# Harounnn/Clustering-Driven-Replication-Strategy

Hardware: AMD Instinct MI355X
Metric: Lloyd point-iters/sec (whole node) + achieved HBM GB/s, 100M files d=16 k=64 (higher is better)
Workload: dtype f64

## Files before the change

clustering-driven-replication-strategy_amd/_cdr.py:

```python
from __future__ import annotations

import ctypes
import os
import sys
import threading

import numpy as np

_HERE = os.path.dirname(os.path.abspath(__file__))
LIB_PATH = os.environ.get("CDR_LIB", os.path.join(_HERE, "libcdr.so"))

CDR_OK = 0
CDR_ERR_ARG = 1
CDR_ERR_HIP = 2
CDR_ERR_NAN = 3
CDR_ERR_STATE = 4
CDR_ERR_UNSUPPORTED = 5
MODE_F32X = 1
MODE_F64 = 2
SEED_BLOCK = 8192
PLAN_SLOT = 64
PLAN_MAX_TAIL = PLAN_SLOT - 1
PLAN_MAX_FIELD = 65535

# ... 7 lines not shown
_PF64 = ctypes.POINTER(ctypes.c_double)

SIGNATURES = {
    "cdr_last_error": ([], ctypes.c_char_p),
    "cdr_version": ([], ctypes.c_int),
    "cdr_device_count": ([ctypes.POINTER(ctypes.c_int)], None),
    "cdr_create": ([ctypes.c_int, ctypes.POINTER(_P)], None),
    "cdr_destroy": ([_P], None),
    "cdr_set_stream": ([_P, _P], None),
    "cdr_synchronize": ([_P], None),
    "cdr_points_load_f64": ([_P, _P, _I64, _I32], None),
    "cdr_points_generate": ([_P, _I64, _I64, _I64, _I32, _I32, _U64], None),
    "cdr_points_info": ([_P, _PI64, _PI32, _PI32, _PI32], None),
    "cdr_points_get_rows": ([_P, _P, _I64, _P], None),
    "cdr_points_stats": ([_P, _P], None),
    "cdr_points_restat": ([_P, _P, _I64], None),
    "cdr_seed_reset": ([_P], None),
    "cdr_seed_update": ([_P, _P], None),
    "cdr_seed_num_blocks": ([_P, _PI64], None),
    "cdr_seed_block_sums": ([_P, _P], None),
    "cdr_seed_scan": ([_P, _F64, _F64, _PF64], None),
    "cdr_seed_search": ([_P, _F64, _F64, _PI64], None),
    "cdr_seed_scan_begin": ([_P, _F64, _F64, _PI64, _PI64], None),
    "cdr_seed_scan_items": ([_P, _P, _I64, _PI64], None),
    "cdr_seed_scan_end": ([_P, _F64, _PF64], None),
    "cdr_seed_program_eval": ([_P, _I64, _F64, _PF64, _PI32], None),
    "cdr_seed_stats": ([_P, _PI64], None),
    "cdr_seed_run": ([_P, _I64, _I32, _P, _P], None),
    "cdr_seed_shard_begin": ([_P, _I64, _I64, _I32, _I32, _I64, _I32, _P, _P, _P], None),
    "cdr_seed_shard_phase": ([_P, _I32, _P, _P], None),
    "cdr_seed_shard_end": ([_P, _P, _P, _P, _P], None),
    "cdr_seed_run_sharded": ([_P, _I64, _I64, _I64, _I32, _P, _P, _P, _P], None),
    "cdr_lloyd_step": ([_P, _P, _I32, _P, _I32], None),
    "cdr_lloyd_step_f64": ([_P, _P, _I32, _P, _P], None),
    "cdr_lloyd_f64_run": ([_P, _P, _I32, _I32, _F64, _P, _P, _P, _P], None),
    "cdr_lloyd_step_f32r": ([_P, _P, _I32, _P, _P], None),
    "cdr_f32r_seed_update": ([_P, _P, _I32, _P], None),
    "cdr_f32r_seed_run": ([_P, _I64, _I32, _P, _P], None),
    "cdr_lloyd_labels": ([_P, _P], None),
    "cdr_lloyd_stats": ([_P, _PI64], None),
    "cdr_debug_screen": ([_P, _P, _I32, _P, _P], None),
    "cdr_debug_plan32": ([_P, _I32, _P, _I32, _P], None),
    "cdr_profile_reset": ([_P, _I32], None),
    "cdr_profile_read": ([_P, _P], None),
    "cdr_profile_read_sub": ([_P, _P], None),
    "cdr_f64s_begin": ([_P, _P, _I32, _I32, _I32, _P, _P], None),
    "cdr_f64s_build": ([_P, _P, _P], None),
    "cdr_f64s_finish": ([_P, _P, _P, _P, _P, _P], None),
    "cdr_f64s_chain": ([_P, _P], None),
    "cdr_profile_kernel": ([_P, _P, _I32], None),
    "cdr_lloyd_screen_layout": ([_P, _P], None),
    "cdr_lloyd_watch_info": ([_P, _P], None),
    "cdr_debug_watch": ([_P, _P, _I64, _P, _I64, _P, _P], None),
    "cdr_lloyd_big_layout": ([_P, _P], None),
    "cdr_debug_big_plan": ([_P, _I32, _P, _I64, _PI64], None),
    "cdr_points_sqdev": ([_P, _P, _PF64], None),
    "cdr_lloyd_begin": ([_P, _P, _I32, _F64, _I32, _P, _F64], None),
    "cdr_lloyd_enqueue_assign": ([_P, _P], None),
    "cdr_lloyd_enqueue_finalize": ([_P, _P], None),
    "cdr_lloyd_status": ([_P, _P, _P], None),
    "cdr_lloyd_read": ([_P, _P, _P, _P], None),
    "cdr_lloyd_resume": ([_P, _P, _I32, _I32], None),
    "cdr_lloyd_end": ([_P], None),
    "cdr_lloyd_enqueue_steps": ([_P, _I32], None),
    "cdr_comm_unique_id": ([_P], None),
    "cdr_comm_init": ([_P, _P, _I32, _I32], None),
    "cdr_comm_destroy": ([_P], None),
    "cdr_comm_available": ([ctypes.POINTER(ctypes.c_int32)], None),
    "cdr_comm_ranks": ([_P, ctypes.POINTER(ctypes.c_int32), ctypes.POINTER(ctypes.c_int32)], None),
    "cdr_build_id": ([], ctypes.c_char_p),
    "cdr_medians_segmented": ([_P, _P, _P, _I64, _P], None),
    "cdr_medians_by_label": ([_P, _I32, _P], None),
    "cdr_features_aggregate": ([_P, _I64, _P, _P, _P, _P, _I64, _P, _P, _PI64], None),
    "cdr_features_finalize": ([_P, _I64, _P, _P, _F64, _P], None),
    "cdr_features_generate": ([_P, _I64, _I64, ctypes.c_uint64, _I64, _I64], None),
    "cdr_features_aggregate_resident": ([_P, _P, _PI64], None),
    "cdr_features_events_read": ([_P, _P, _P, _P, _P, _P], None),
    "cdr_features_groupby_info": ([_P, _P], None),
    "cdr_lloyd_f64_walked": ([_P, _PI64], None),
    "cdr_medians_group": ([_P, _I32, _P], None),
    "cdr_medians_begin": ([_P, _P, ctypes.POINTER(ctypes.c_int32), _PI64], None),
    "cdr_medians_pass_hist": ([_P, _I32, _P], None),
    "cdr_medians_pass_select": ([_P, _I32, _P], None),
    "cdr_medians_finish": ([_P, _P], None),
    "cdr_medians_global": ([_P, _P], None),
    "cdr_medians_global_begin": ([_P, _I64, ctypes.POINTER(ctypes.c_int32), _PI64], None),
    "cdr_medians_global_pass_hist": ([_P, _I32, _P], None),
    "cdr_medians_global_pass_select": ([_P, _I32, _P], None),
    "cdr_medians_global_finish": ([_P, _P], None),
    "cdr_medians_global_timing": ([_P, _P], None),
    "cdr_features_exchange_pack": ([_P, _I32, _P, _P, _P, _PI64], None),
    "cdr_features_exchange_unpack": ([_P, _P, _I64, _I64, _I64], None),
    "cdr_features_load_events": ([_P, _I64, _P, _P, _P, _P, _I64, _P], None),
    "cdr_features_finalize_stats": ([_P, _I64, _P, _P, ctypes.c_double, _P, _P], None),
    "cdr_features_finalize_apply": ([_P, _I64, _P, _P, ctypes.c_double, _P, _P, _I64, _P],
                                    None),
    "cdr_features_simulate": ([_P, _I64, _I64, ctypes.c_double, _I32, ctypes.c_uint64, _I64,
                               _PI64], None),
    "cdr_ingest_manifest": ([_P, _I64, _P, _P, _P, _I32, _P, _P], None),
    "cdr_ingest_log": ([_P, _P, _I64, _P], None),
    "cdr_ingest_reparse": ([_P, _P], None),
    "cdr_quality_silhouette": ([_P, _P, _I64, _P, _I32, _P, _P, _P], None),
    "cdr_quality_scatter": ([_P, _P, _I32, _P, _P, _P], None),
    "cdr_quality_timing": ([_P, _P], None),
    "cdr_csv_format": ([_P, _I64, _I32, ctypes.c_uint32, _P, _P, _P, _P, _I64, _PI64, _P, _I64,
                        _PI64], None),
# ... 384 lines not shown
        out = np.empty(self.info()["n"], dtype=np.int64)
        _check(self._lib.cdr_lloyd_labels(self._h, _ptr(out)))
        return out

    def fallback_count(self) -> int:
        v = _I64()
        _check(self._lib.cdr_lloyd_stats(self._h, ctypes.byref(v)))
        return int(v.value)

    def profile_reset(self, enable: bool = True, every: int = 1) -> None:
        _check(self._lib.cdr_profile_reset(self._h, max(int(every), 1) if enable else 0))

    def profile_read(self) -> dict:
        out = np.zeros(6, dtype=np.float64)
        _check(self._lib.cdr_profile_read(self._h, _ptr(out)))
        return {"screen_ms": out[0], "steps": int(out[1]), "step_ms": out[2],
                "fallback_points": int(out[3]), "queued_points": int(out[4]),
                "tight_points": int(out[5])}

    def profile_read_sub(self) -> dict:
        out = np.zeros(2, dtype=np.float64)
        _check(self._lib.cdr_profile_read_sub(self._h, _ptr(out)))
        return {"first_ms": out[0], "steps": int(out[1])}

    def profile_kernel(self) -> str:
        buf = ctypes.create_string_buffer(96)
        _check(self._lib.cdr_profile_kernel(self._h, buf, 96))
        return buf.value.decode()

    def screen_layout(self) -> dict:
        out = np.zeros(6, dtype=np.int32)
        _check(self._lib.cdr_lloyd_screen_layout(self._h, _ptr(out)))
        names = ("workgroups", "slot_wg", "dyn_pct", "max_chunks", "nchunks", "word_bytes")
        return {nm: int(v) for nm, v in zip(names, out)}

    def watch_info(self) -> dict:
        out = np.zeros(12, dtype=np.int64)
        _check(self._lib.cdr_lloyd_watch_info(self._h, _ptr(out)))
        names = ("mode", "listed", "failed", "epochs", "full_steps", "list_steps", "waves",
                 "range", "cap", "next_list", "carried", "n_pad")
        return {nm: int(v) for nm, v in zip(names, out)}

    def debug_watch(self) -> dict:
        info = self.watch_info()
        words = np.zeros(info["n_pad"], dtype=np.uint16)
        entries = np.zeros((info["waves"], info["cap"]), dtype=np.uint32)
        counts = np.zeros(info["waves"], dtype=np.int32)
        tables = np.zeros((3, 64), dtype=np.uint32)
        _check(self._lib.cdr_debug_watch(self._h, _ptr(words), words.size, _ptr(entries),
                                         entries.size, _ptr(counts), _ptr(tables)))
        return {"words": words, "entries": entries, "counts": counts, "T": tables[0],
                "H": tables[1], "HL": tables[2], **info}

    def big_layout(self) -> dict:
        out = np.zeros(15, dtype=np.int64)
        _check(self._lib.cdr_lloyd_big_layout(self._h, _ptr(out)))
        names = ("DQ", "KB", "FG", "JB", "l1_threads", "l2_form", "delta", "plan", "regions",
                 "cap1", "groups", "leftovers", "l3", "mv1", "mv2")
        return {nm: int(v) for nm, v in zip(names, out)}

    def debug_big_plan(self, k: int) -> dict:
        d = self.info()["d"]
        dq, kb = -(-d // 16), -(-int(k) // 32)
        b1, bc, bC = kb * dq * 64 * 16, kb * 32 * 4, 8 * int(k) * d
        got = _I64()
        _check(self._lib.cdr_debug_big_plan(self._h, int(k), None, 0, ctypes.byref(got)))
        if got.value != b1 + bc + bC + 16:
            raise RuntimeError(f"debug_big_plan: {got.value} bytes, expected {b1 + bc + bC + 16}")
        raw = np.empty(got.value, dtype=np.uint8)
        _check(self._lib.cdr_debug_big_plan(self._h, int(k), _ptr(raw), raw.size,
                                            ctypes.byref(got)))
        return {"frag1": raw[:b1].copy(), "cinit": raw[b1:b1 + bc].copy(),
                "C": raw[b1 + bc:b1 + bc + bC].copy().view(np.float64).reshape(int(k), d),
                "thr": raw[b1 + bc + bC:b1 + bc + bC + 8].copy().view(np.float32)}

    LL_RUNNING, LL_CONVERGED, LL_EMPTY, LL_HOST_PLAN, LL_AMBIGUOUS = 0, 1, 2, 3, 4

    def points_sqdev(self, ref) -> float:
        ref = np.ascontiguousarray(ref, dtype=np.float64)
        v = _F64()
        _check(self._lib.cdr_points_sqdev(self._h, _ptr(ref), ctypes.byref(v)))
        return float(v.value)

    def lloyd_begin(self, C, tol: float, ref, x2_total: float = float("nan"),
                    round32: bool = False) -> None:
        C = np.ascontiguousarray(C, dtype=np.float64)
        ref = np.ascontiguousarray(ref, dtype=np.float64)
        self._ll_shape = C.shape
        _check(self._lib.cdr_lloyd_begin(self._h, _ptr(C), C.shape[0], float(tol),
                                         1 if round32 else 0, _ptr(ref), float(x2_total)))

    def lloyd_enqueue_assign(self, dsums_ptr: int | None = None) -> None:
        _check(self._lib.cdr_lloyd_enqueue_assign(self._h, _P(dsums_ptr or 0)))

    def lloyd_enqueue_finalize(self, dsums_ptr: int | None = None) -> None:
        _check(self._lib.cdr_lloyd_enqueue_finalize(self._h, _P(dsums_ptr or 0)))

    def lloyd_status(self) -> dict:
        st = np.zeros(4, dtype=np.int64)
        v = np.zeros(2, dtype=np.float64)
        _check(self._lib.cdr_lloyd_status(self._h, _ptr(st), _ptr(v)))
        return {"running": bool(st[0]), "steps": int(st[1]), "reason": int(st[2]),
                "enqueued": int(st[3]), "shift": float(v[0]), "inertia": float(v[1])}

    def lloyd_read(self):
        k, d = self._ll_shape
# ... 588 lines not shown
```

clustering-driven-replication-strategy_amd/csrc/loop.hip:

```cpp
#include <cmath>
#include <cstdio>
#include <cstring>

#include "cdr_internal.h"
#include "fin32.h"
#include "plan32.h"

namespace cdr {

constexpr int kLLState = 8;

void plan32_point_side(const Ctx& c, double& xxmax, double& l1x);
void zh_rebase(Ctx& c, const long long* gate);
constexpr int kRebaseEvery = 4;

constexpr int kFinThreads = 512;
constexpr int kFinLds = 64 * 17;

__global__ __launch_bounds__(kFinThreads) void ll_finalize(FinArgs a) {
  long long* __restrict__ state = a.state;
  const int k = a.k, d = a.d;
  double* __restrict__ C = a.C;
  double* __restrict__ Cnew = a.Cnew;
  const int cells = k * (d + 1);
  __shared__ long long lsum[kFinLds];
  __shared__ double lC[kFinLds];
  __shared__ double lref[2 * 64];
  const bool staged = cells <= kFinLds && d <= 64;
  const double* __restrict__ ref = staged ? lref : a.ref;
  const double* __restrict__ Cin = staged ? lC : C;
  if (staged) {
    constexpr int PER = (kFinLds + kFinThreads - 1) / kFinThreads;
    long long p[PER][kRunSlices];
    double cv[PER];
    double rv = 0.0;
    const long long st0 = state[0];
#pragma unroll
    for (int i = 0; i < PER; ++i) {
      const int c = threadIdx.x + i * kFinThreads;
#pragma unroll
      for (int sl = 0; sl < kRunSlices; ++sl)
        p[i][sl] = (c < cells && sl < a.nslices) ? a.sums[(size_t)sl * cells + c] : 0;
      cv[i] = c < k * d ? C[c] : 0.0;
    }
    if (threadIdx.x < 2 * d) rv = a.ref[threadIdx.x];
    if (st0 == 0) return;
#pragma unroll
    for (int i = 0; i < PER; ++i) {
      const int c = threadIdx.x + i * kFinThreads;
      long long v = 0;
#pragma unroll
      for (int sl = 0; sl < kRunSlices; ++sl) v += p[i][sl];
      if (c < cells) lsum[c] = v;
      if (c < k * d) lC[c] = cv[i];
    }
    if (threadIdx.x < 2 * d) lref[threadIdx.x] = rv;
    __syncthreads();
  } else if (state[0] == 0) {
    return;
  }
  auto sum_at = [&](size_t e) -> long long {
    if (staged) return lsum[e];
    long long v = 0;
    for (int sl = 0; sl < a.nslices; ++sl) v += a.sums[(size_t)sl * cells + e];
    return v;
  };
// ... 483 lines not shown
  int wh[16];
  HIP_CHECK(hipMemcpy(wh, static_cast<unsigned char*>(c.bnd.p) + kBndWatch, sizeof(wh),
                      hipMemcpyDeviceToHost));
  std::vector<int32_t> wn((size_t)c.watch_waves), wf((size_t)c.watch_waves);
  HIP_CHECK(hipMemcpy(wn.data(), c.wn.p, sizeof(int32_t) * wn.size(), hipMemcpyDeviceToHost));
  HIP_CHECK(hipMemcpy(wf.data(), c.wf.p, sizeof(int32_t) * wf.size(), hipMemcpyDeviceToHost));
  const bool any = wh[kWListN] + wh[kWFullN] > 0;
  out[0] = any ? wh[kWLast] : -1;
  if (wh[kWEpochs] > 0)
    for (int32_t v : wn) out[1] += v;
  if (any)
    for (int32_t v : wf) out[2] += v;
  out[3] = wh[kWEpochs];
  out[4] = wh[kWFullN];
  out[5] = wh[kWListN];
  out[6] = c.watch_waves;
  out[7] = c.watch_range;
  out[8] = c.watch_cap;
  out[9] = wh[kWMode] == kWatchList && wh[kWOvf] == 0 ? 1 : 0;
  out[10] = wh[kWCarried];
  CDR_CATCH
}

int cdr_debug_watch(cdr_ctx* h, uint16_t* words, int64_t n_words, uint32_t* entries,
                    int64_t n_entries, int32_t* counts, uint32_t* tables) {
  CDR_TRY
  if (!h) CDR_FAIL(CDR_ERR_ARG, "null ctx");
  Ctx& c = h->c;
  if (!c.watch_on || !c.zb_valid || c.zb_fmt != 16)
    CDR_FAIL(CDR_ERR_STATE, "watch list: the list path is not on");
  if ((words && n_words != c.n_pad) ||
      (entries && n_entries != (int64_t)c.watch_waves * c.watch_cap))
    CDR_FAIL(CDR_ERR_ARG, "watch list: buffer sizes differ from cdr_lloyd_watch_info's");
  HIP_CHECK(hipSetDevice(c.device));
  HIP_CHECK(hipStreamSynchronize(c.stream));
  if (words)
    HIP_CHECK(hipMemcpy(words, c.zb.p, sizeof(uint16_t) * (size_t)c.n_pad, hipMemcpyDeviceToHost));
  if (entries)
    HIP_CHECK(hipMemcpy(entries, c.wl.p,
                        sizeof(uint32_t) * (size_t)c.watch_waves * (size_t)c.watch_cap,
                        hipMemcpyDeviceToHost));
  if (counts)
    HIP_CHECK(hipMemcpy(counts, c.wn.p, sizeof(int32_t) * (size_t)c.watch_waves,
                        hipMemcpyDeviceToHost));
  if (tables) {
    const unsigned char* bt = static_cast<const unsigned char*>(c.bnd.p);
    HIP_CHECK(hipMemcpy(tables, bt + kBndT, 256, hipMemcpyDeviceToHost));
    HIP_CHECK(hipMemcpy(tables + 64, bt + kBndH, 256, hipMemcpyDeviceToHost));
    HIP_CHECK(hipMemcpy(tables + 128, bt + kBndHL, 256, hipMemcpyDeviceToHost));
  }
  CDR_CATCH
}

int cdr_lloyd_end(cdr_ctx* h) {
  CDR_TRY
  if (!h) CDR_FAIL(CDR_ERR_ARG, "null ctx");
  h->c.ll_on = false;
  CDR_CATCH
}

}
```

clustering-driven-replication-strategy_amd/csrc/screen32_common.h:

```cpp
#pragma once
#include <type_traits>
#include <cstdio>
#include <cmath>
#include <cstring>
#include <algorithm>
#include <vector>

#include "cdr_internal.h"
#include "exact_math.h"
#include "plan32.h"

namespace cdr {

typedef _Float16 h8 __attribute__((ext_vector_type(8)));
typedef _Float16 h16 __attribute__((ext_vector_type(16)));
typedef float f4 __attribute__((ext_vector_type(4)));
typedef float f16v __attribute__((ext_vector_type(16)));
typedef _Float16 h2 __attribute__((ext_vector_type(2)));

__device__ __forceinline__ unsigned pack_h2(float a, float b) {
  h2 h = {(_Float16)a, (_Float16)b};
  return __builtin_bit_cast(unsigned, h);
}

// ... 213 lines not shown
  const float s = (l0 - u0) + w;
  const float m = 0x1p-21f * ((l0 + u0) + w);
  const float z = s - m;
  return (z > 0.0f ? (__float_as_uint(z) & ~63u) : 0xBF800000u) | label;
}

__device__ __forceinline__ unsigned short zb16_pack(float l0, float u0, float w, int e0,
                                                    unsigned label) {
  if (!(l0 > 0.0f) || !(u0 >= 0.0f) || !(w >= 0.0f)) return (unsigned short)label;
  l0 = fminf(l0, 0x1p60f) * (1.0f - 0x1p-20f);
  const float s = (l0 - u0) + w;
  const float m = 0x1p-21f * ((l0 + u0) + w);
  int c = zb16_code(s - m, e0);
  c = c < 0 ? 0 : (c > 1022 ? 1022 : c);
  return (unsigned short)((unsigned)c << 6 | label);
}


template <int QMAX, class F>
inline void dispatch_q_mt(int Q, int MT, F&& f) {
  static_assert(QMAX == 2 || QMAX == 4, "feature quads: 1..2 per lane half or 1..4 per point");
  if (Q < 1 || Q > QMAX || MT < 1 || MT > 2)
    CDR_FAIL(CDR_ERR_STATE, "screen32: no kernel for this (Q, MT)");
  auto with_q = [&](auto q) {
    if (MT == 1) f(q, std::integral_constant<int, 1>{});
    else f(q, std::integral_constant<int, 2>{});
  };
  if constexpr (QMAX == 4) {
    if (Q == 3) return with_q(std::integral_constant<int, 3>{});
    if (Q == 4) return with_q(std::integral_constant<int, 4>{});
  }
  if (Q == 1) with_q(std::integral_constant<int, 1>{});
  else with_q(std::integral_constant<int, 2>{});
}

template <class K>
inline int occupancy_blocks(K kernel, size_t lds) {
  int nb = 0;
  if (hipOccupancyMaxActiveBlocksPerMultiprocessor(&nb, kernel, 256, lds) != hipSuccess || nb < 1)
    nb = 2;
  return nb > 8 ? 8 : nb;
}

int screen32_blocks_per_cu(int QH, int MT, size_t lds);
void screen32_launch(int QH, int MT, dim3 grid, hipStream_t s, size_t lds, const S32Args& a);
int screen32p_blocks_per_cu(int Q, int MT);
void screen32p_launch(int Q, int MT, dim3 grid, hipStream_t s, const S32PArgs& p);
int screen32b_blocks_per_cu(int Q, int MT);
void screen32b_launch(int Q, int MT, dim3 grid, hipStream_t s, const S32BArgs& p);
void screen32bz_launch(dim3 grid, hipStream_t s, const S32BArgs& p);
void bound_words_reset(bool z16, hipStream_t s, const uint8_t* lab8, void* zb, int64_t n,
                       int64_t n_pad, const long long* gate);
void zh_rebase(Ctx& c, const long long* gate);
int screen32bs_blocks_per_cu(int Q, int MT, bool list);
void screen32bs_launch(int Q, int MT, dim3 grid, hipStream_t s, const S32BArgs& p, bool split);

}
```

clustering-driven-replication-strategy_amd/csrc/screen32b.hip:

```cpp
#include "screen32_common.h"
#include "screen32_fix.h"

namespace cdr {

template <int Q, int MT>
__global__ __launch_bounds__(256, 4) void screen32b(S32BArgs B) {
  const S32PArgs& a = B.p;
  constexpr int QH = FixDims<Q>::QH;
  if (a.gate && a.gate[0] == 0) return;
  constexpr bool H1 = QH == 1;
  constexpr int kTile = H1 ? 512 : 1024;
  constexpr int kHalf = kTile / 2;
  constexpr int kPB = H1 ? 8 : 16;
  constexpr int NWH = kPB / 4;
  constexpr int kRow = 2 * kPB;
  typedef unsigned u4v __attribute__((ext_vector_type(4)));
  __shared__ __attribute__((aligned(16))) float c32s[64 * kPrStr + 128];
  float* const eb = c32s + 64 * kPrStr;
  float* const hc = eb + 64;
  constexpr size_t kQBytes = 4 * 2 * 2 * kTile + 4 * 128 * sizeof(int2);
  __shared__ __attribute__((aligned(16))) unsigned char qlds[kQBytes > kFixLdsBytes ? kQBytes : kFixLdsBytes];
  typedef unsigned char QRow[2][2 * kTile];
  QRow* qd = reinterpret_cast<QRow*>(qlds);
  int2 (*qm)[128] = reinterpret_cast<int2 (*)[128]>(qlds + 4 * 2 * 2 * kTile);
// ... 383 lines not shown
  if (lane < cnt) out[total + lane] = fl[lane];
  if (lane == 0) B.zn[wave] = total + cnt;
}

__global__ void zb_reset_kernel(const uint8_t* __restrict__ lab8, uint32_t* __restrict__ zb,
                                int64_t n, int64_t n_pad, const long long* __restrict__ gate) {
  if (gate && gate[0] == 0) return;
  for (int64_t i = (int64_t)blockIdx.x * blockDim.x + threadIdx.x; i < n_pad;
       i += (int64_t)gridDim.x * blockDim.x)
    zb[i] = i < n ? (kZbStale | lab8[i]) : 0x7F000000u;
}

__global__ void zh_reset_kernel(const uint8_t* __restrict__ lab8, uint16_t* __restrict__ zh,
                                int64_t n, int64_t n_pad, const long long* __restrict__ gate) {
  if (gate && gate[0] == 0) return;
  for (int64_t i = (int64_t)blockIdx.x * blockDim.x + threadIdx.x; i < n_pad;
       i += (int64_t)gridDim.x * blockDim.x)
    zh[i] = i < n ? (uint16_t)lab8[i] : (uint16_t)kZ16Pad;
}

__device__ __forceinline__ unsigned zb16_rebase(unsigned w, float dg, int e0o, int e0n) {
  const unsigned c = w >> 6;
  if (c == 0u || c == 1023u) return w;
  const float t = zb16_dec((int)c, e0o) - dg;
  int cn = t > 0.0f ? zb16_code(t * (1.0f - 0x1p-22f), e0n) : -1;
  cn = cn < 0 ? 0 : (cn > 1022 ? 1022 : cn);
  return (unsigned)cn << 6 | (w & 63u);
}

__global__ __launch_bounds__(256) void zh_rebase_kernel(uint16_t* __restrict__ zh, int64_t n_pad,
                                                        const unsigned char* __restrict__ bt,
                                                        const long long* __restrict__ gate) {
  if (gate && gate[0] == 0) return;
  const int* hd = reinterpret_cast<const int*>(bt + kBndHdr);
  if (hd[3] == 0) return;
  __shared__ float dgs[64];
  if (threadIdx.x < 64) dgs[threadIdx.x] = reinterpret_cast<const float*>(bt + kBndDG)[threadIdx.x];
  __syncthreads();
  const int e0o = hd[1], e0n = hd[2];
  typedef unsigned u4v __attribute__((ext_vector_type(4)));
  u4v* z4 = reinterpret_cast<u4v*>(zh);
  for (int64_t i = (int64_t)blockIdx.x * blockDim.x + threadIdx.x; i < n_pad / 8;
       i += (int64_t)gridDim.x * blockDim.x) {
    u4v z = __builtin_nontemporal_load(z4 + i);
#pragma unroll
    for (int q = 0; q < 4; ++q) {
      const unsigned lo = z[q] & 0xFFFFu, hi = z[q] >> 16;
      z[q] = zb16_rebase(lo, dgs[lo & 63u], e0o, e0n) | zb16_rebase(hi, dgs[hi & 63u], e0o, e0n) << 16;
    }
    __builtin_nontemporal_store(z, z4 + i);
  }
}

__global__ __launch_bounds__(256) void zh_watch_kernel(uint16_t* __restrict__ zh, int64_t n_pad,
                                                       unsigned char* __restrict__ bt,
                                                       const long long* __restrict__ gate,
                                                       uint32_t* __restrict__ wl,
                                                       int32_t* __restrict__ wn, int wcap,
                                                       int wrange) {
  if (gate && gate[0] == 0) return;
  const int* hd = reinterpret_cast<const int*>(bt + kBndHdr);
  int* wh = reinterpret_cast<int*>(bt + kBndWatch);
  const bool reb = hd[3] != 0;
  if (!reb && (wh[kWFin] == kWatchList || wh[kWHold])) return;
  __shared__ float dgs[64];
  __shared__ unsigned hs[64];
  const int t = threadIdx.x, lane = t & 63;
  if (t < 64) {
    dgs[t] = reinterpret_cast<const float*>(bt + kBndDG)[t];
    hs[t] = reinterpret_cast<const unsigned*>(bt + kBndH)[t];
  }
  __syncthreads();
  if (blockIdx.x == 0) {
    if (t < 64) reinterpret_cast<unsigned*>(bt + kBndHL)[t] = hs[t];
    if (t == 0) {
      wh[kWMode] = kWatchList;
      wh[kWValid] = 1;
      wh[kWEpochs] += 1;
      if (reb) wh[kWCarried] += 1;
    }
  }
  const int e0o = hd[1], e0n = hd[2];
  typedef unsigned u4v __attribute__((ext_vector_type(4)));
  const int wave = blockIdx.x * 4 + (t >> 6);
  const int64_t p0 = (int64_t)wave * wrange;
  const int64_t p1 = p0 + wrange < n_pad ? p0 + wrange : n_pad;
  uint32_t* const out = wl + (size_t)wave * wcap;
  int cnt = 0;
  constexpr int kU = 4;
  for (int64_t c0 = p0; c0 < p1; c0 += kU * kZ16Chunk) {
    u4v z[kU];
#pragma unroll
    for (int i = 0; i < kU; ++i) {
      const int64_t ci = c0 + i * kZ16Chunk < p1 ? c0 + i * kZ16Chunk : c0;
      z[i] = __builtin_nontemporal_load(reinterpret_cast<const u4v*>(zh + ci) + lane);
    }
#pragma unroll
    for (int i = 0; i < kU; ++i) {
      const int64_t ci = c0 + i * kZ16Chunk;
      if (ci >= p1) break;
      if (reb) {
#pragma unroll
        for (int q = 0; q < 4; ++q) {
          const unsigned lo = z[i][q] & 0xFFFFu, hi = z[i][q] >> 16;
          z[i][q] = zb16_rebase(lo, dgs[lo & 63u], e0o, e0n) |
                    zb16_rebase(hi, dgs[hi & 63u], e0o, e0n) << 16;
        }
        __builtin_nontemporal_store(z[i], reinterpret_cast<u4v*>(zh + ci) + lane);
      }
      const unsigned off = (unsigned)(ci - p0) + 8u * (unsigned)lane;
#pragma unroll
      for (int u = 0; u < 8; ++u) {
        const unsigned w = (z[i][u >> 1] >> (16 * (u & 1))) & 0xFFFFu;
        const bool listed = (w >> 6) <= hs[w & 63u];
        const unsigned long long m = __ballot(listed);
        if (m) {
          const int r = cnt + __builtin_amdgcn_mbcnt_hi((unsigned)(m >> 32),
                                                        __builtin_amdgcn_mbcnt_lo((unsigned)m, 0u));
          if (listed && r < wcap) out[r] = (off + (unsigned)u) << 16 | w;
          cnt += __popcll(m);
        }
      }
    }
  }
  if (lane == 0) {
    wn[wave] = cnt < wcap ? cnt : wcap;
    if (cnt > wcap) wh[kWOvf] = 1;
  }
}

void zh_rebase(Ctx& c, const long long* gate) {
  if (!c.zb_valid || c.zb_fmt != 16 || !c.bnd_ok) return;
  if (c.watch_on)
    hipLaunchKernelGGL(zh_watch_kernel, dim3(c.watch_waves / 4), dim3(256), 0, c.stream,
                       c.zb.as<uint16_t>(), c.n_pad, static_cast<unsigned char*>(c.bnd.p), gate,
                       c.wl.as<uint32_t>(), c.wn.as<int32_t>(), c.watch_cap, c.watch_range);
  else
    hipLaunchKernelGGL(zh_rebase_kernel, dim3(2048), dim3(256), 0, c.stream, c.zb.as<uint16_t>(),
                       c.n_pad, reinterpret_cast<const unsigned char*>(c.bnd.p), gate);
  HIP_CHECK(hipGetLastError());
}

void bound_words_reset(bool z16, hipStream_t s, const uint8_t* lab8, void* zb, int64_t n,
                       int64_t n_pad, const long long* gate) {
  if (z16)
    hipLaunchKernelGGL(zh_reset_kernel, dim3(2048), dim3(256), 0, s, lab8,
                       static_cast<uint16_t*>(zb), n, n_pad, gate);
  else
    hipLaunchKernelGGL(zb_reset_kernel, dim3(2048), dim3(256), 0, s, lab8,
                       static_cast<uint32_t*>(zb), n, n_pad, gate);
}

int screen32b_blocks_per_cu(int Q, int MT) {
  static int cache[4][2] = {};
  int& nb = cache[Q - 1][MT - 1];
  if (!nb)
    dispatch_q_mt<4>(Q, MT, [&](auto q, auto m) {
      nb = occupancy_blocks(screen32b<decltype(q)::value, decltype(m)::value>, 0);
    });
  return nb;
}

void screen32b_launch(int Q, int MT, dim3 grid, hipStream_t s, const S32BArgs& p) {
  dispatch_q_mt<4>(Q, MT, [&](auto q, auto m) {
    hipLaunchKernelGGL((screen32b<decltype(q)::value, decltype(m)::value>), grid, dim3(256), 0, s, p);
  });
}

void screen32bz_launch(dim3 grid, hipStream_t s, const S32BArgs& p) {
  static const int pd = exp_env("CDR_S32BZ_PD") ? std::atoi(exp_env("CDR_S32BZ_PD")) : 8;
  if (pd == 4) hipLaunchKernelGGL(screen32bz<4>, grid, dim3(256), 0, s, p);
  else if (pd == 12) hipLaunchKernelGGL(screen32bz<12>, grid, dim3(256), 0, s, p);
  else hipLaunchKernelGGL(screen32bz<8>, grid, dim3(256), 0, s, p);
}

}
```

include/cdr.h:

```cpp
#ifndef CDR_H_
#define CDR_H_

#include <stdint.h>

#ifdef __cplusplus
extern "C" {
#endif

#define CDR_OK 0
#define CDR_ERR_ARG 1
#define CDR_ERR_HIP 2
#define CDR_ERR_NAN 3
#define CDR_ERR_STATE 4
#define CDR_ERR_UNSUPPORTED 5

#define CDR_MODE_F32X 1
#define CDR_MODE_F64 2

typedef struct cdr_ctx cdr_ctx;

const char* cdr_last_error(void);
int cdr_version(void);
int cdr_device_count(int* out);

// ... 46 lines not shown
                         int32_t rank, int64_t first, int32_t k, const double* u, double* red,
                         int64_t* sizes);
int cdr_seed_shard_phase(cdr_ctx* ctx, int32_t phase, const void* in, void* out);
int cdr_seed_shard_end(cdr_ctx* ctx, const double* red, int64_t* picks, double* centres,
                       int32_t* status);
int cdr_seed_run_sharded(cdr_ctx* ctx, int64_t row_begin, int64_t n_total, int64_t first, int32_t k,
                         const double* u, int64_t* picks, double* centres, int32_t* status);
int cdr_seed_program_eval(const cdr_seed_item* items, int64_t n_items, double c_in,
                          double* c_out, int32_t* ok);
int cdr_seed_search(cdr_ctx* ctx, double c_last, double u, int64_t* idx);

int cdr_lloyd_step(cdr_ctx* ctx, const double* C, int32_t k, int64_t* out,
                   int32_t out_on_device);
int cdr_lloyd_step_f64(cdr_ctx* ctx, const double* C, int32_t k, double* sums,
                       int64_t* counts);
int cdr_lloyd_f64_run(cdr_ctx* ctx, const double* C, int32_t k, int32_t max_steps, double tol,
                      double* C_out, double* means_out, int64_t* counts_out, int32_t* info);
int cdr_lloyd_step_f32r(cdr_ctx* ctx, const float* C, int32_t k, double* sums,
                        int64_t* counts);
int cdr_lloyd_f64_walked(cdr_ctx* ctx, int64_t* walked);
int cdr_f64s_begin(cdr_ctx* ctx, const double* C, int32_t k, int32_t nranks, int32_t rank,
                   void* tot_buf, int64_t* sizes);
int cdr_f64s_build(cdr_ctx* ctx, const void* tot_buf, void* prog_buf);
int cdr_f64s_finish(cdr_ctx* ctx, const void* tot_buf, const void* prog_buf, double* sums,
                    int64_t* counts, int32_t* status);
int cdr_f64s_chain(cdr_ctx* ctx, void* chain_buf);
int cdr_lloyd_labels(cdr_ctx* ctx, int64_t* labels);
int cdr_lloyd_stats(cdr_ctx* ctx, int64_t* n_fallback);
int cdr_profile_reset(cdr_ctx* ctx, int32_t enable);
int cdr_profile_read(cdr_ctx* ctx, double* out);
int cdr_profile_read_sub(cdr_ctx* ctx, double* out);

int cdr_points_sqdev(cdr_ctx* ctx, const double* ref, double* out);
int cdr_lloyd_begin(cdr_ctx* ctx, const double* C, int32_t k, double tol, int32_t flags,
                    const double* ref, double x2_total);
int cdr_lloyd_enqueue_assign(cdr_ctx* ctx, int64_t* dsums);
int cdr_lloyd_enqueue_finalize(cdr_ctx* ctx, const int64_t* dsums);
int cdr_lloyd_status(cdr_ctx* ctx, int64_t* status, double* values);
int cdr_lloyd_read(cdr_ctx* ctx, double* C, double* means, int64_t* counts);
int cdr_lloyd_resume(cdr_ctx* ctx, const double* C, int32_t add_steps, int32_t host_plan_once);
int cdr_lloyd_end(cdr_ctx* ctx);
int cdr_lloyd_enqueue_steps(cdr_ctx* ctx, int32_t m);

int cdr_comm_unique_id(void* id128);
int cdr_comm_init(cdr_ctx* ctx, const void* id128, int32_t nranks, int32_t rank);
int cdr_comm_destroy(cdr_ctx* ctx);
int cdr_comm_available(int32_t* ok);
int cdr_comm_ranks(cdr_ctx* ctx, int32_t* nranks, int32_t* rank);
int cdr_profile_kernel(cdr_ctx* ctx, char* buf, int32_t len);
int cdr_lloyd_screen_layout(cdr_ctx* ctx, int32_t out[6]);
int cdr_lloyd_watch_info(cdr_ctx* ctx, int64_t out[12]);
int cdr_debug_watch(cdr_ctx* ctx, uint16_t* words, int64_t n_words, uint32_t* entries,
                    int64_t n_entries, int32_t* counts, uint32_t* tables);
int cdr_lloyd_big_layout(cdr_ctx* ctx, int64_t out[15]);
int cdr_debug_screen(cdr_ctx* ctx, const double* C, int32_t k, float* out_vals,
                     float* thr_a0a1);
int cdr_debug_plan32(cdr_ctx* ctx, int32_t which, const double* C, int32_t k, float* out);
int cdr_debug_big_plan(cdr_ctx* ctx, int32_t k, void* out, int64_t bytes, int64_t* written);

int cdr_medians_segmented(cdr_ctx* ctx, const double* values,
                          const int64_t* offsets, int64_t n_segments,
                          double* out);
int cdr_medians_by_label(cdr_ctx* ctx, int32_t k, double* out);
int cdr_medians_group(cdr_ctx* ctx, int32_t k, int64_t* counts);
int cdr_medians_begin(cdr_ctx* ctx, const int64_t* global_counts, int32_t* passes,
                      int64_t* hist_words);
int cdr_medians_pass_hist(cdr_ctx* ctx, int32_t pass, void* hist);
int cdr_medians_pass_select(cdr_ctx* ctx, int32_t pass, const void* hist);
int cdr_medians_finish(cdr_ctx* ctx, double* out);

int cdr_medians_global(cdr_ctx* ctx, double* out );
int cdr_medians_global_begin(cdr_ctx* ctx, int64_t n_total, int32_t* passes,
                             int64_t* hist_words);
int cdr_medians_global_pass_hist(cdr_ctx* ctx, int32_t pass, void* hist);
int cdr_medians_global_pass_select(cdr_ctx* ctx, int32_t pass, const void* hist);
int cdr_medians_global_finish(cdr_ctx* ctx, double* out);
int cdr_medians_global_timing(cdr_ctx* ctx, double* out);

int cdr_features_aggregate(cdr_ctx* ctx, int64_t n_events,
                           const int32_t* file_idx, const uint8_t* op,
                           const int32_t* client, const int64_t* ts_us,
                           int64_t n_files, const int32_t* primary,
                           int64_t* out, int64_t* max_ts_us);
int cdr_features_generate(cdr_ctx* ctx, int64_t n_events, int64_t n_files, uint64_t seed,
                          int64_t t0_us, int64_t span_us);
int cdr_features_aggregate_resident(cdr_ctx* ctx, int64_t* out, int64_t* max_ts_us);
int cdr_features_simulate(cdr_ctx* ctx, int64_t n_files, int64_t file_begin, double duration_s,
                          int32_t n_clients, uint64_t seed, int64_t t0_us, int64_t* n_events);
int cdr_features_events_read(cdr_ctx* ctx, int32_t* file_idx, uint8_t* op, int32_t* client,
                             int64_t* ts_us, int32_t* primary);
int cdr_features_groupby_info(cdr_ctx* ctx, int64_t* info);
int cdr_features_exchange_pack(cdr_ctx* ctx, int32_t nranks, const int64_t* bounds, void* send,
                               int64_t* counts, int64_t* max_ts_us);
int cdr_features_exchange_unpack(cdr_ctx* ctx, const void* recv, int64_t n, int64_t file_begin,
                                 int64_t file_end);
int cdr_features_load_events(cdr_ctx* ctx, int64_t n, const int32_t* file_idx, const uint8_t* op,
                             const int32_t* client, const int64_t* ts_us, int64_t n_files,
                             const int32_t* primary);
int cdr_features_finalize_stats(cdr_ctx* ctx, int64_t n_rows, const int64_t* counts,
                                const double* creation_s, double observation_end,
                                int64_t* istats, double* dstats);
int cdr_features_finalize_apply(cdr_ctx* ctx, int64_t n_rows, const int64_t* counts,
                                const double* creation_s, double observation_end,
                                const int64_t* istats, const double* dstats,
                                int64_t n_rows_total, double* out);
int cdr_ingest_manifest(cdr_ctx* ctx, int64_t n_files, const char* path_bytes,
// ... 66 lines not shown
```

Baseline: 2753 billion.

## Stream watch-list build with deep prefetch and LDS ring-buffered coalesced writes

```diff
diff --git a/clustering-driven-replication-strategy_amd/_cdr.py b/clustering-driven-replication-strategy_amd/_cdr.py
--- a/clustering-driven-replication-strategy_amd/_cdr.py
+++ b/clustering-driven-replication-strategy_amd/_cdr.py
@@ -83,6 +83,8 @@
     "cdr_lloyd_screen_layout": ([_P, _P], None),
     "cdr_lloyd_watch_info": ([_P, _P], None),
     "cdr_debug_watch": ([_P, _P, _I64, _P, _I64, _P, _P], None),
+    "cdr_debug_watch_build": ([_P, _P, _I64, _P, _P, _I32, _I32, _I32, _I32, _I32, _P, _P, _P,
+                               _P], None),
     "cdr_lloyd_big_layout": ([_P, _P], None),
     "cdr_debug_big_plan": ([_P, _I32, _P, _I64, _PI64], None),
     "cdr_points_sqdev": ([_P, _P, _PF64], None),
@@ -573,6 +575,29 @@
         return {"words": words, "entries": entries, "counts": counts, "T": tables[0],
                 "H": tables[1], "HL": tables[2], **info}
 
+    def debug_watch_build(self, words, H, waves: int, wrange: int, cap: int, rebase=None,
+                          fill: int = 0) -> dict:
+        words = np.array(words, dtype=np.uint16)
+        H = np.ascontiguousarray(H, dtype=np.uint32)
+        if H.size != 64:
+            raise ValueError("H: 64 codes")
+        entries = np.full((int(waves), int(cap)), fill, dtype=np.uint32)
+        counts = np.zeros(int(waves), dtype=np.int32)
+        ovf = np.zeros(1, dtype=np.int32)
+        dG, e0o, e0n, rebased = None, 0, 0, None
+        if rebase is not None:
+            dG = np.ascontiguousarray(rebase[0], dtype=np.float32)
+            if dG.size != 64:
+                raise ValueError("dG: 64 floats")
+            e0o, e0n = int(rebase[1]), int(rebase[2])
+            rebased = np.zeros_like(words)
+        _check(self._lib.cdr_debug_watch_build(
+            self._h, _ptr(words), words.size, _ptr(H), _ptr(dG) if dG is not None else None,
+            e0o, e0n, int(waves), int(wrange), int(cap), _ptr(entries), _ptr(counts), _ptr(ovf),
+            _ptr(rebased) if rebased is not None else None))
+        return {"words": words, "entries": entries, "counts": counts, "overflow": int(ovf[0]),
+                "rebased": rebased}
+
     def big_layout(self) -> dict:
         out = np.zeros(15, dtype=np.int64)
         _check(self._lib.cdr_lloyd_big_layout(self._h, _ptr(out)))
diff --git a/clustering-driven-replication-strategy_amd/csrc/loop.hip b/clustering-driven-replication-strategy_amd/csrc/loop.hip
--- a/clustering-driven-replication-strategy_amd/csrc/loop.hip
+++ b/clustering-driven-replication-strategy_amd/csrc/loop.hip
@@ -12,6 +12,9 @@
 
 void plan32_point_side(const Ctx& c, double& xxmax, double& l1x);
 void zh_rebase(Ctx& c, const long long* gate);
+void zh_watch_build_debug(Ctx& c, uint16_t* words, int64_t n_pad, const uint32_t* H,
+                          const float* dG, int e0o, int e0n, int waves, int wrange, int wcap,
+                          uint32_t* entries, int32_t* counts, int32_t* ovf, uint16_t* rebased);
 constexpr int kRebaseEvery = 4;
 
 constexpr int kFinThreads = 512;
@@ -601,6 +604,20 @@
   CDR_CATCH
 }
 
+int cdr_debug_watch_build(cdr_ctx* h, uint16_t* words, int64_t n_words, const uint32_t* H,
+                          const float* dG, int32_t e0_old, int32_t e0_new, int32_t waves,
+                          int32_t range, int32_t cap, uint32_t* entries, int32_t* counts,
+                          int32_t* overflow, uint16_t* rebased) {
+  CDR_TRY
+  if (!h || !words || !H || !entries || !counts || !overflow)
+    CDR_FAIL(CDR_ERR_ARG, "null argument");
+  Ctx& c = h->c;
+  HIP_CHECK(hipSetDevice(c.device));
+  zh_watch_build_debug(c, words, n_words, H, dG, e0_old, e0_new, waves, range, cap, entries,
+                       counts, overflow, rebased);
+  CDR_CATCH
+}
+
 int cdr_lloyd_end(cdr_ctx* h) {
   CDR_TRY
   if (!h) CDR_FAIL(CDR_ERR_ARG, "null ctx");
diff --git a/clustering-driven-replication-strategy_amd/csrc/screen32_common.h b/clustering-driven-replication-strategy_amd/csrc/screen32_common.h
--- a/clustering-driven-replication-strategy_amd/csrc/screen32_common.h
+++ b/clustering-driven-replication-strategy_amd/csrc/screen32_common.h
@@ -289,6 +289,9 @@
 void bound_words_reset(bool z16, hipStream_t s, const uint8_t* lab8, void* zb, int64_t n,
                        int64_t n_pad, const long long* gate);
 void zh_rebase(Ctx& c, const long long* gate);
+void zh_watch_build_debug(Ctx& c, uint16_t* words, int64_t n_pad, const uint32_t* H,
+                          const float* dG, int e0o, int e0n, int waves, int wrange, int wcap,
+                          uint32_t* entries, int32_t* counts, int32_t* ovf, uint16_t* rebased);
 int screen32bs_blocks_per_cu(int Q, int MT, bool list);
 void screen32bs_launch(int Q, int MT, dim3 grid, hipStream_t s, const S32BArgs& p, bool split);
 
diff --git a/clustering-driven-replication-strategy_amd/csrc/screen32b.hip b/clustering-driven-replication-strategy_amd/csrc/screen32b.hip
--- a/clustering-driven-replication-strategy_amd/csrc/screen32b.hip
+++ b/clustering-driven-replication-strategy_amd/csrc/screen32b.hip
@@ -459,6 +459,81 @@
   }
 }
 
+constexpr int kWbPD = 8;
+constexpr int kWbRing = 1024;
+template <bool REB>
+__device__ __forceinline__ int zh_watch_stream(uint16_t* __restrict__ zh, int64_t p0, int nch,
+                                               const float* dgs, const unsigned* hw, int e0o,
+                                               int e0n, uint32_t* ring, uint32_t* __restrict__ out,
+                                               int wcap, int lane) {
+  typedef unsigned u4v __attribute__((ext_vector_type(4)));
+  if (nch <= 0) return 0;
+  u4v* const zw = reinterpret_cast<u4v*>(zh + p0) + lane;
+  auto zload = [&](u4v& z, int ci) __attribute__((always_inline)) {
+    z = __builtin_nontemporal_load(zw + (size_t)(ci < nch ? ci : nch - 1) * 64);
+  };
+  u4v zc[kWbPD];
+#pragma unroll
+  for (int i = 0; i < kWbPD - 1; ++i) zload(zc[i], i);
+  int cnt = 0, tail = 0;
+  for (int c0 = 0; c0 < nch; c0 += kWbPD) {
+#pragma unroll
+    for (int i = 0; i < kWbPD; ++i) {
+      const int ci = c0 + i;
+      if (ci >= nch) break;
+      zload(zc[(i + kWbPD - 1) % kWbPD], ci + kWbPD - 1);
+      u4v z = zc[i];
+      if (REB) {
+#pragma unroll
+        for (int q = 0; q < 4; ++q) {
+          const unsigned lo = z[q] & 0xFFFFu, hi = z[q] >> 16;
+          z[q] = zb16_rebase(lo, dgs[lo & 63u], e0o, e0n) |
+                 zb16_rebase(hi, dgs[hi & 63u], e0o, e0n) << 16;
+        }
+        __builtin_nontemporal_store(z, zw + (size_t)ci * 64);
+      }
+      unsigned wd[8];
+      bool ls[8];
+      unsigned c = 0;
+#pragma unroll
+      for (int u = 0; u < 8; ++u) {
+        wd[u] = u & 1 ? z[u >> 1] >> 16 : z[u >> 1] & 0xFFFFu;
+        ls[u] = wd[u] <= hw[wd[u] & 63u];
+        c += ls[u];
+      }
+      int pre = 0, tot = 0;
+#pragma unroll
+      for (int b = 0; b < 4; ++b) {
+        const unsigned long long m = __ballot((c >> b) & 1u);
+        pre += __builtin_amdgcn_mbcnt_hi((unsigned)(m >> 32),
+                                         __builtin_amdgcn_mbcnt_lo((unsigned)m, 0u)) << b;
+        tot += __popcll(m) << b;
+      }
+      if (tot == 0) continue;
+      if (cnt < wcap) {
+        const unsigned off16 = ((unsigned)ci * kZ16Chunk + 8u * (unsigned)lane) << 16;
+        int r = cnt + pre;
+#pragma unroll
+        for (int u = 0; u < 8; ++u)
+          if (ls[u]) ring[r++ & (kWbRing - 1)] = off16 | (unsigned)u << 16 | wd[u];
+      }
+      cnt += tot;
+      __builtin_amdgcn_wave_barrier();
+#pragma unroll
+      for (int k = 0; k < 2; ++k)
+        if (tail + 256 <= cnt && tail < wcap) {
+          const u4v e = *reinterpret_cast<const u4v*>(ring + (tail & (kWbRing - 1)) + 4 * lane);
+          *reinterpret_cast<u4v*>(out + tail + 4 * lane) = e;
+          tail += 256;
+        }
+      __builtin_amdgcn_wave_barrier();
+    }
+  }
+  __builtin_amdgcn_wave_barrier();
+  for (int o = tail + lane; o < (cnt < wcap ? cnt : wcap); o += 64) out[o] = ring[o & (kWbRing - 1)];
+  return cnt;
+}
+
 __global__ __launch_bounds__(256) void zh_watch_kernel(uint16_t* __restrict__ zh, int64_t n_pad,
                                                        unsigned char* __restrict__ bt,
                                                        const long long* __restrict__ gate,
@@ -471,11 +546,13 @@
   const bool reb = hd[3] != 0;
   if (!reb && (wh[kWFin] == kWatchList || wh[kWHold])) return;
   __shared__ float dgs[64];
-  __shared__ unsigned hs[64];
+  __shared__ unsigned hs[64], hw[64];
+  __shared__ __attribute__((aligned(16))) uint32_t ring[4][kWbRing];
   const int t = threadIdx.x, lane = t & 63;
   if (t < 64) {
     dgs[t] = reinterpret_cast<const float*>(bt + kBndDG)[t];
     hs[t] = reinterpret_cast<const unsigned*>(bt + kBndH)[t];
+    hw[t] = hs[t] << 6 | (unsigned)t;
   }
   __syncthreads();
   if (blockIdx.x == 0) {
@@ -488,48 +565,14 @@
     }
   }
   const int e0o = hd[1], e0n = hd[2];
-  typedef unsigned u4v __attribute__((ext_vector_type(4)));
-  const int wave = blockIdx.x * 4 + (t >> 6);
+  const int wv = __builtin_amdgcn_readfirstlane(t >> 6);
+  const int wave = blockIdx.x * 4 + wv;
   const int64_t p0 = (int64_t)wave * wrange;
   const int64_t p1 = p0 + wrange < n_pad ? p0 + wrange : n_pad;
+  const int nch = p1 > p0 ? (int)((p1 - p0) / kZ16Chunk) : 0;
   uint32_t* const out = wl + (size_t)wave * wcap;
-  int cnt = 0;
-  constexpr int kU = 4;
-  for (int64_t c0 = p0; c0 < p1; c0 += kU * kZ16Chunk) {
-    u4v z[kU];
-#pragma unroll
-    for (int i = 0; i < kU; ++i) {
-      const int64_t ci = c0 + i * kZ16Chunk < p1 ? c0 + i * kZ16Chunk : c0;
-      z[i] = __builtin_nontemporal_load(reinterpret_cast<const u4v*>(zh + ci) + lane);
-    }
-#pragma unroll
-    for (int i = 0; i < kU; ++i) {
-      const int64_t ci = c0 + i * kZ16Chunk;
-      if (ci >= p1) break;
-      if (reb) {
-#pragma unroll
-        for (int q = 0; q < 4; ++q) {
-          const unsigned lo = z[i][q] & 0xFFFFu, hi = z[i][q] >> 16;
-          z[i][q] = zb16_rebase(lo, dgs[lo & 63u], e0o, e0n) |
-                    zb16_rebase(hi, dgs[hi & 63u], e0o, e0n) << 16;
-        }
-        __builtin_nontemporal_store(z[i], reinterpret_cast<u4v*>(zh + ci) + lane);
-      }
-      const unsigned off = (unsigned)(ci - p0) + 8u * (unsigned)lane;
-#pragma unroll
-      for (int u = 0; u < 8; ++u) {
-        const unsigned w = (z[i][u >> 1] >> (16 * (u & 1))) & 0xFFFFu;
-        const bool listed = (w >> 6) <= hs[w & 63u];
-        const unsigned long long m = __ballot(listed);
-        if (m) {
-          const int r = cnt + __builtin_amdgcn_mbcnt_hi((unsigned)(m >> 32),
-                                                        __builtin_amdgcn_mbcnt_lo((unsigned)m, 0u));
-          if (listed && r < wcap) out[r] = (off + (unsigned)u) << 16 | w;
-          cnt += __popcll(m);
-        }
-      }
-    }
-  }
+  const int cnt = reb ? zh_watch_stream<true>(zh, p0, nch, dgs, hw, e0o, e0n, ring[wv], out, wcap, lane)
+                      : zh_watch_stream<false>(zh, p0, nch, dgs, hw, e0o, e0n, ring[wv], out, wcap, lane);
   if (lane == 0) {
     wn[wave] = cnt < wcap ? cnt : wcap;
     if (cnt > wcap) wh[kWOvf] = 1;
@@ -548,6 +591,55 @@
   HIP_CHECK(hipGetLastError());
 }
 
+void zh_watch_build_debug(Ctx& c, uint16_t* words, int64_t n_pad, const uint32_t* H,
+                          const float* dG, int e0o, int e0n, int waves, int wrange, int wcap,
+                          uint32_t* entries, int32_t* counts, int32_t* ovf, uint16_t* rebased) {
+  if (n_pad <= 0 || n_pad % kZ16Chunk || waves <= 0 || waves % 4 || wrange <= 0 ||
+      wrange % kZ16Chunk || wrange > kS32WatchMaxRange || wcap <= 0 || wcap % 256 || wcap > wrange ||
+      (int64_t)waves * wrange < n_pad)
+    CDR_FAIL(CDR_ERR_ARG, "watch build: whole chunks, waves in fours, regions of whole 256-entry "
+                          "blocks within a range of at most 65536 points, every point in a range");
+  const size_t wb = sizeof(uint16_t) * (size_t)n_pad, eb = sizeof(uint32_t) * (size_t)waves * wcap;
+  DevBuf zh, zr, bt, wl, wn;
+  struct Free {
+    DevBuf *a, *b, *c, *d, *e;
+    ~Free() {
+      for (DevBuf* p : {a, b, c, d, e}) p->release();
+    }
+  } guard{&zh, &zr, &bt, &wl, &wn};
+  zh.ensure(wb);
+  bt.ensure(kBndBytes);
+  wl.ensure(eb);
+  wn.ensure(sizeof(int32_t) * (size_t)waves);
+  std::vector<unsigned char> hb(kBndBytes, 0);
+  const int hdr[4] = {1, e0o, e0n, dG ? 1 : 0};
+  std::memcpy(hb.data() + kBndHdr, hdr, sizeof(hdr));
+  std::memcpy(hb.data() + kBndH, H, 256);
+  if (dG) std::memcpy(hb.data() + kBndDG, dG, 256);
+  HIP_CHECK(hipMemcpyAsync(zh.p, words, wb, hipMemcpyHostToDevice, c.stream));
+  HIP_CHECK(hipMemcpyAsync(bt.p, hb.data(), kBndBytes, hipMemcpyHostToDevice, c.stream));
+  HIP_CHECK(hipMemcpyAsync(wl.p, entries, eb, hipMemcpyHostToDevice, c.stream));
+  HIP_CHECK(hipMemsetAsync(wn.p, 0xFF, sizeof(int32_t) * (size_t)waves, c.stream));
+  if (dG) {
+    zr.ensure(wb);
+    HIP_CHECK(hipMemcpyAsync(zr.p, words, wb, hipMemcpyHostToDevice, c.stream));
+    hipLaunchKernelGGL(zh_rebase_kernel, dim3(2048), dim3(256), 0, c.stream, zr.as<uint16_t>(),
+                       n_pad, static_cast<const unsigned char*>(bt.p), nullptr);
+  }
+  hipLaunchKernelGGL(zh_watch_kernel, dim3(waves / 4), dim3(256), 0, c.stream, zh.as<uint16_t>(),
+                     n_pad, static_cast<unsigned char*>(bt.p), nullptr, wl.as<uint32_t>(),
+                     wn.as<int32_t>(), wcap, wrange);
+  HIP_CHECK(hipGetLastError());
+  HIP_CHECK(hipMemcpyAsync(words, zh.p, wb, hipMemcpyDeviceToHost, c.stream));
+  HIP_CHECK(hipMemcpyAsync(entries, wl.p, eb, hipMemcpyDeviceToHost, c.stream));
+  HIP_CHECK(hipMemcpyAsync(counts, wn.p, sizeof(int32_t) * (size_t)waves, hipMemcpyDeviceToHost,
+                           c.stream));
+  HIP_CHECK(hipMemcpyAsync(hb.data(), bt.p, kBndBytes, hipMemcpyDeviceToHost, c.stream));
+  if (dG && rebased) HIP_CHECK(hipMemcpyAsync(rebased, zr.p, wb, hipMemcpyDeviceToHost, c.stream));
+  HIP_CHECK(hipStreamSynchronize(c.stream));
+  *ovf = reinterpret_cast<const int*>(hb.data() + kBndWatch)[kWOvf];
+}
+
 void bound_words_reset(bool z16, hipStream_t s, const uint8_t* lab8, void* zb, int64_t n,
                        int64_t n_pad, const long long* gate) {
   if (z16)
diff --git a/include/cdr.h b/include/cdr.h
--- a/include/cdr.h
+++ b/include/cdr.h
@@ -122,6 +122,10 @@
 int cdr_lloyd_watch_info(cdr_ctx* ctx, int64_t out[12]);
 int cdr_debug_watch(cdr_ctx* ctx, uint16_t* words, int64_t n_words, uint32_t* entries,
                     int64_t n_entries, int32_t* counts, uint32_t* tables);
+int cdr_debug_watch_build(cdr_ctx* ctx, uint16_t* words, int64_t n_words, const uint32_t* H,
+                          const float* dG, int32_t e0_old, int32_t e0_new, int32_t waves,
+                          int32_t range, int32_t cap, uint32_t* entries, int32_t* counts,
+                          int32_t* overflow, uint16_t* rebased);
 int cdr_lloyd_big_layout(cdr_ctx* ctx, int64_t out[15]);
 int cdr_debug_screen(cdr_ctx* ctx, const double* C, int32_t k, float* out_vals,
                      float* thr_a0a1);
```

After: 2753 billion. No clear change (-0.0%).
